# TravisWheelerLab/BATH

Hardware: AMD Instinct MI355X
Metric: DP Gcells/s + residues/s through bathsearch pipeline at 1/2/4/8 MI355X (higher is better)
Workload: dtype u8/i16 integer scores (SSV: exact binary16), f32 Forward

## Files before the change

### bath_amd/csrc/bath_pipeline.hip

```cpp
#include <algorithm>
#include <cmath>
#include <cstring>
#include <cstdlib>
#include <map>
#include <thread>

#include "bath_common.hpp"
#include "bath_kernels.hpp"
#include "bath_launch.hpp"
#include "host_model.hpp"

using namespace bath;

namespace bath {

static const double kLog2 = 0.69314718055994529;

enum { FLAG_VIT_RUN = 1, FLAG_HAS_WIN = 2 };

struct Counters {
  int cand_count, todo_msv, todo_vit, todo_ssvb, todo_vit2, todo_fwd, win_count, overflow;
  int todo_lb;
  int fwd_next;
  unsigned long long n_orfs, orf_res;
  unsigned long long n_past_msv, n_past_bias, n_past_vit, n_past_fwd;
  unsigned long long pos_past_msv, pos_past_bias, pos_past_vit, pos_past_fwd;
  unsigned long long res_vit, res_fwd;
  unsigned long long res_seen;
};

struct Params {
  double F1, F2, F3, F4;
  int do_bias, fs_pipe, minlen;
  float evparam[BATH_NEVPARAM];
};

template <int NR, int G>
__global__ __launch_bounds__(256, NR <= 76 ? 4 : 1) void ssv_orf_kernel(const uint8_t *__restrict__ aa, const OrfRec *__restrict__ orfs, const int *__restrict__ n_orfs_dev,
                                                      SeqView dna, const int16_t *__restrict__ cost_tab, int row_bytes,
                                                      const int16_t *__restrict__ emit_thresh, int thresh_max,
                                                      Cand cand, int cand_cap, Counters *__restrict__ ctr) {
  extern __shared__ __attribute__((aligned(16))) char lds[];
  {
    const int n32 = kSsvRows * row_bytes / 4;
    const uint32_t *src = reinterpret_cast<const uint32_t *>(cost_tab);
    uint32_t *dst = reinterpret_cast<uint32_t *>(lds);
    for (int i = threadIdx.x; i < n32; i += blockDim.x) dst[i] = src[i];
  }
  __syncthreads();
  constexpr int TPW = 64 / G;
  const int64_t n_orfs = *n_orfs_dev;
  const int lane = threadIdx.x & 63;
  const int grank = SsvGroups<G>::rank(lane);
  const char *tile = lds + grank * (4 * NR);
  const unsigned tile_addr = (unsigned)(size_t)(__attribute__((address_space(3))) const char *)tile;
  const int64_t wave0 = ((int64_t)blockIdx.x * blockDim.x + threadIdx.x) >> 6;
  const int64_t nwaves = ((int64_t)gridDim.x * blockDim.x) >> 6;
  const s16x2 fl = {0, 0};
  for (int64_t tb = wave0 * TPW; tb < n_orfs; tb += nwaves * TPW) {
    const int64_t t = tb + SsvGroups<G>::slot(lane);
    const bool live = t < n_orfs;
    OrfRec rec{0, 0, 0};
    if (live) rec = orfs[t];
    const int L = rec.len_sf & 0x0fffffff;
    const uint8_t *s = aa + rec.aa_off;
    const int Lw = wave_max_i32(L);
    s16x2 reg[NR];
#pragma unroll
    for (int r = 0; r < NR; r++) reg[r] = fl;
    s16x2 xE = fl, xE2 = fl;
    uint64_t qnext = (0 < L) ? *reinterpret_cast<const uint64_t *>(s) : 0x1d1d1d1d1d1d1d1dull;
    for (int i0 = 0; i0 < Lw; i0 += 8) {
      const uint64_t q = qnext;
      qnext = (i0 + 8 < L) ? *reinterpret_cast<const uint64_t *>(s + i0 + 8) : 0x1d1d1d1d1d1d1d1dull;
      const int nrow = min(8, Lw - i0);
      for (int h = 0; h < 2; h++) {
        const uint32_t qh = h ? (uint32_t)(q >> 32) : (uint32_t)q;
        const int nh = min(4, nrow - 4 * h);
        for (int j = 0; j < nh; j++) {
          int x = (int)__builtin_amdgcn_ubfe(qh, 8 * j, 8);
          x = (i0 + 4 * h + j < L) ? x : kRowReset;
          const unsigned carry = ssv_carry<NR, G>(reg, grank);
          ssv_row_pipe<NR, 3>(reg, xE, xE2, tile_addr + __umul24((unsigned)x, (unsigned)row_bytes), carry);
        }
      }
    }
    xE = ssv_max3(xE, xE2, xE2);
    const int v = ssv_group_max<G>(xE);
    if (dna.context) {
      unsigned long long r = 0;
      if (live && grank == 0) {
        const int sf = (int)((unsigned)rec.len_sf >> 28);
        const int64_t w = rec.w;
        const int startj = (int32_t)(rec.aa_off - (2 * dna.off[w] + 96 * w + (int64_t)sf * orf_stream_pitch(dna.len[w])));
        const int C = dna.context[w], start_s = sf % 3 + 3 * startj + 1;
        if (sf < 3 ? (start_s + 3 * L - 1 < C) : (dna.len[w] - start_s + 1 < C)) r = (unsigned long long)L;
      }
      if (__ballot(r != 0)) { for (int d = 32; d >= 1; d >>= 1) r += __shfl_xor(r, d, 64); if (lane == 0) atomicAdd(&ctr->res_seen, r); }
    }
    if (live && grank == 0 && v >= (int)emit_thresh[min(L, thresh_max)]) {
      const int sf = (int)((unsigned)rec.len_sf >> 28);
      const int64_t w = rec.w;
      const int64_t stream = 2 * dna.off[w] + 96 * w + (int64_t)sf * orf_stream_pitch(dna.len[w]);
      const int startj = (int32_t)(rec.aa_off - stream);
      bool seen = false;
      if (dna.context) {
        const int C = dna.context[w], start_s = sf % 3 + 3 * startj + 1;
        seen = sf < 3 ? (start_s + 3 * L - 1 < C) : (dna.len[w] - start_s + 1 < C);
      }
      const int slot = seen ? cand_cap + 1 : atomicAdd(&ctr->cand_count, 1);
      if (seen) {
      } else if (slot < cand_cap) {
        cand.window[slot] = w; cand.sf[slot] = sf; cand.startj[slot] = startj; cand.len[slot] = L;
        cand.v[slot] = (int16_t)min(v, 32767); cand.off[slot] = rec.aa_off;
      } else atomicOr(&ctr->overflow, 1);
    }
  }
}

__device__ __forceinline__ double d_gumbel_surv(double x, double mu, double lambda) {
  const double ey = -exp(-lambda * (x - mu));
  if (fabs(ey) < 5e-9) return -ey;
  return 1.0 - exp(ey);
}
__device__ __forceinline__ double d_exp_surv(double x, double mu, double lambda) { return (x < mu) ? 1.0 : exp(-lambda * (x - mu)); }

__device__ __forceinline__ int cand_classify(const Cand &cand, int c, int tjb, const MsvConsts &mc) {
  float sc = 0.f;
  const int st = ssv_classify(cand.v[c], tjb, mc, &sc);
  cand.usc[c] = sc; cand.msv_status[c] = st; cand.stage[c] = 0; cand.flags[c] = 0;
  cand.vfsc[c] = -INFINITY; cand.fwdsc[c] = -INFINITY; cand.vit_status[c] = 0; cand.filtersc[c] = 0.f; cand.P[c] = 1.0;
  cand.kminmax[2 * c] = 1 << 30; cand.kminmax[2 * c + 1] = 0;
  return st;
}

template <int NL, int NS, int CAP>
struct BlockTally {
  int n[NL > 0 ? NL : 1], base[NL > 0 ? NL : 1];
  unsigned long long sum[NS > 0 ? NS : 1];
  int32_t ids[NL > 0 ? NL : 1][NL > 0 ? CAP : 1];
};
template <int NL, int NS>
struct TallyOut {
  int32_t *list[NL > 0 ? NL : 1]; int *count[NL > 0 ? NL : 1];
  unsigned long long *sum[NS > 0 ? NS : 1];
};
template <int NL, int NS, int CAP>
__device__ __forceinline__ void tally_reset(BlockTally<NL, NS, CAP> &t) {
  if ((int)threadIdx.x < NL) t.n[threadIdx.x] = 0;
  if ((int)threadIdx.x < NS) t.sum[threadIdx.x] = 0ull;
  __syncthreads();
}
template <int NL, int NS, int CAP>
__device__ __forceinline__ void tally_add(BlockTally<NL, NS, CAP> &t, int k, unsigned long long v) { atomicAdd(&t.sum[k], v); }
template <int NL, int NS, int CAP>
__device__ __forceinline__ void tally_push(BlockTally<NL, NS, CAP> &t, int l, int32_t id) { t.ids[l][atomicAdd(&t.n[l], 1)] = id; }
template <int NL, int NS, int CAP>
__device__ __forceinline__ bool tally_lists_full(BlockTally<NL, NS, CAP> &t) {
  bool full = false;
  __syncthreads();
#pragma unroll
  for (int l = 0; l < NL; l++) full |= t.n[l] > CAP - (int)blockDim.x;
  __syncthreads();
  return full;
}
template <int NL, int NS, int CAP>
__device__ __forceinline__ void tally_write_lists(BlockTally<NL, NS, CAP> &t, const TallyOut<NL, NS> &o) {
  if (NL == 0) return;
  __syncthreads();
#pragma unroll
  for (int l = 0; l < NL; l++) if ((int)threadIdx.x == l && t.n[l] > 0) t.base[l] = atomicAdd(o.count[l], t.n[l]);
  __syncthreads();
#pragma unroll
  for (int l = 0; l < NL; l++) {
    const int n = t.n[l], b = t.base[l];
    for (int i = threadIdx.x; i < n; i += blockDim.x) o.list[l][b + i] = t.ids[l][i];
  }
  __syncthreads();
  if ((int)threadIdx.x < NL) t.n[threadIdx.x] = 0;
  __syncthreads();
}
template <int NL, int NS, int CAP>
__device__ __forceinline__ void tally_finish(BlockTally<NL, NS, CAP> &t, const TallyOut<NL, NS> &o) {
  tally_write_lists(t, o);
  if (NL == 0) __syncthreads();
#pragma unroll
  for (int k = 0; k < NS; k++) if ((int)threadIdx.x == k && t.sum[k] != 0ull) atomicAdd(o.sum[k], t.sum[k]);
}

__global__ __launch_bounds__(256) void classify_kernel(Cand cand, int cand_cap, Counters *__restrict__ ctr, const uint8_t *__restrict__ tjb_tab, MsvConsts mc,
                                                       int32_t *__restrict__ todo_msv) {
  __shared__ BlockTally<1, 0, 512> tally;
  tally_reset(tally);
  const TallyOut<1, 0> out{{todo_msv}, {&ctr->todo_msv}, {nullptr}};
  const int ncand = min(ctr->cand_count, cand_cap);
  for (int c0 = blockIdx.x * blockDim.x; c0 < ncand; c0 += gridDim.x * blockDim.x) {
    if (tally_lists_full(tally)) tally_write_lists(tally, out);
    const int c = c0 + threadIdx.x;
    if (c < ncand && cand_classify(cand, c, tjb_tab[cand.len[c]], mc) == BATH_ENORESULT) tally_push(tally, 0, c);
  }
  tally_finish(tally, out);
}

struct F1Tables { const float *eo, *nullsc, *p1, *lt1, *lt2; };
enum { F1_TODO_VIT = 0, F1_TODO_SSVB = 1, F1_NL = 2 };
enum { F1_N_MSV = 0, F1_POS_MSV, F1_N_BIAS, F1_POS_BIAS, F1_RES_VIT, F1_NS };
__device__ __forceinline__ TallyOut<F1_NL, F1_NS> f1_tally_out(Counters *__restrict__ ctr, int32_t *__restrict__ todo_vit, int32_t *__restrict__ todo_ssvb) {
  return TallyOut<F1_NL, F1_NS>{{todo_vit, todo_ssvb}, {&ctr->todo_vit, &ctr->todo_ssvb},
                                {&ctr->n_past_msv, &ctr->pos_past_msv, &ctr->n_past_bias, &ctr->pos_past_bias, &ctr->res_vit}};
}
template <int CAP>
__device__ __forceinline__ void cand_f1_bias(const Cand &cand, int c, BlockTally<F1_NL, F1_NS, CAP> &tally, const Params &p, const uint8_t *__restrict__ pool, int M,
                                             const float *s_eo , const F1Tables &t) {
  const int L = cand.len[c];
  const float usc = cand.usc[c];
  const float nullsc = t.nullsc[L];
  cand.nullsc[c] = nullsc;
  float seqsc = (float)((double)(usc - nullsc) / kLog2);
  double P = d_gumbel_surv(seqsc, p.evparam[0], p.evparam[1]);
  cand.P[c] = P;
  if (P > p.F1) return;
  tally_add(tally, F1_N_MSV, 1ull); tally_add(tally, F1_POS_MSV, (unsigned long long)L * 3ull);
  cand.stage[c] = 1;
  float filtersc = nullsc;
  if (p.do_bias) {
    filtersc = bias_forward(pool + cand.off[c], L, M, s_eo, t.p1[L]);
    filtersc = (filtersc + t.lt1[L]) + t.lt2[L];
    seqsc = (float)((double)(usc - filtersc) / kLog2);
    P = d_gumbel_surv(seqsc, p.evparam[0], p.evparam[1]);
    cand.P[c] = P; cand.filtersc[c] = filtersc;
    if (P > p.F1) return;
  }
  cand.filtersc[c] = filtersc;
  tally_add(tally, F1_N_BIAS, 1ull); tally_add(tally, F1_POS_BIAS, (unsigned long long)L * 3ull);
  cand.stage[c] = 2;
  if (P > p.F2) { cand.flags[c] |= FLAG_VIT_RUN; tally_push(tally, F1_TODO_VIT, c); tally_add(tally, F1_RES_VIT, (unsigned long long)L); }
  else tally_push(tally, F1_TODO_SSVB, c);
}

__global__ __launch_bounds__(256) void f1_bias_kernel(Cand cand, int cand_cap, Counters *__restrict__ ctr, Params p, const uint8_t *__restrict__ pool, int M, F1Tables t,
                                                      int32_t *__restrict__ todo_vit, int32_t *__restrict__ todo_ssvb) {
  __shared__ float s_eo[kKp * 2];
  __shared__ BlockTally<F1_NL, F1_NS, 512> tally;
  for (int i = threadIdx.x; i < kKp * 2; i += blockDim.x) s_eo[i] = t.eo[i];
  tally_reset(tally);
  const TallyOut<F1_NL, F1_NS> out = f1_tally_out(ctr, todo_vit, todo_ssvb);
  const int ncand = min(ctr->cand_count, cand_cap);
  for (int c0 = blockIdx.x * blockDim.x; c0 < ncand; c0 += gridDim.x * blockDim.x) {
    if (tally_lists_full(tally)) tally_write_lists(tally, out);
    const int c = c0 + threadIdx.x;
    if (c < ncand) cand_f1_bias(cand, c, tally, p, pool, M, s_eo, t);
  }
  tally_finish(tally, out);
}

template <int NR>
__global__ __launch_bounds__(256, 4) void msv_stage_kernel(Cand cand, int cand_cap, Counters *__restrict__ ctr,
                                                           const int16_t *__restrict__ cost_tab , int row_bytes,
                                                           const uint8_t *__restrict__ tjb_tab, MsvConsts mc, Params p, const uint8_t *__restrict__ pool, int M,
                                                           F1Tables t, int32_t *__restrict__ todo_vit, int32_t *__restrict__ todo_ssvb) {
  extern __shared__ __attribute__((aligned(16))) char lds[];
  __shared__ float s_eo[kKp * 2];
  __shared__ BlockTally<F1_NL, F1_NS, 256> tally;
  const int ncand = min(ctr->cand_count, cand_cap);
  if ((int64_t)blockIdx.x * blockDim.x >= ncand) return;
  {
    const int n32 = kSsvRows * row_bytes / 4;
    const uint32_t *src = reinterpret_cast<const uint32_t *>(cost_tab);
    uint32_t *dst = reinterpret_cast<uint32_t *>(lds);
    for (int i = threadIdx.x; i < n32; i += blockDim.x) dst[i] = src[i];
    for (int i = threadIdx.x; i < kKp * 2; i += blockDim.x) s_eo[i] = t.eo[i];
  }
  tally_reset(tally);
  const int64_t job = (int64_t)blockIdx.x * blockDim.x + threadIdx.x;
  const bool live = job < ncand;
  const int c = live ? (int)job : 0;
  const int L = live ? cand.len[c] : 0;
  const int tjb = tjb_tab[L];
  const bool rescore = live && cand_classify(cand, c, tjb, mc) == BATH_ENORESULT;
  const int Lr = rescore ? L : 0;
  const uint8_t *s = pool + (rescore ? cand.off[c] : 0);
  bool overflow = false;
  const int xJ = msv_lane_rows<NR>(lds, row_bytes, s, Lr, wave_max_i32(Lr), (uint8_t)((int8_t)tjb + (int8_t)mc.tbm), mc, &overflow);
  if (rescore) {
    if (overflow) { cand.usc[c] = INFINITY; cand.msv_status[c] = BATH_ERANGE; }
    else { cand.usc[c] = msv_lane_score(xJ, tjb, mc); cand.msv_status[c] = BATH_OK; }
  }
  if (live) cand_f1_bias(cand, c, tally, p, pool, M, s_eo, t);
  tally_finish(tally, f1_tally_out(ctr, todo_vit, todo_ssvb));
}

template <int C>
__global__ __launch_bounds__(256) void ssv_bath_kernel(Cand cand, const Counters *__restrict__ ctr, const int32_t *__restrict__ todo,
                                                       const uint8_t *__restrict__ pool, int M, const uint8_t *__restrict__ rb, int rb_stride,
                                                       const uint8_t *__restrict__ ssv_scores, const uint8_t *__restrict__ tjb_tab,
                                                       const float *__restrict__ nullsc_tab, MsvConsts mc, double invP_f1,
                                                       WindowRec *__restrict__ wins, int win_cap, Counters *__restrict__ ctrw) {
  const int lane = threadIdx.x & 63;
  const int64_t wid = ((int64_t)blockIdx.x * blockDim.x + threadIdx.x) >> 6;
  const int64_t nw = ((int64_t)gridDim.x * blockDim.x) >> 6;
  const int ntodo = ctr->todo_ssvb;
  const int Q = max(2, ((M - 1) / 16) + 1);
  for (int64_t job = wid; job < ntodo; job += nw) {
    const int c = todo[job];
    const int L = cand.len[c];
    const uint8_t *s = pool + cand.off[c];
    const int tjb = tjb_tab[L];
    const float nullsc = nullsc_tab[L];
    const int sc_thresh = (uint8_t)(int)ceil((((double)nullsc + ((double)(float)invP_f1 * kLog2) + 3.0) * (double)mc.scale_b) + mc.base + mc.tec + tjb);
    const int tjbm = (uint8_t)((int8_t)tjb + (int8_t)mc.tbm);
    const int xB = satu8(mc.base - tjbm);
    int kmin = 1 << 30, kmax = 0;
    int dp[C];
#pragma unroll
    for (int k = 0; k < C; k++) dp[k] = 0;
    const int ph = threadIdx.x & 63;
    int rbuf = (ph < L) ? (int)s[ph] : 0, rnext = 0;
    for (int i = 1; i <= L; i++) {
      const int j = (i - 1) & 63;
      if (j == 0) { const int q = i - 1 + 64 + ph; rnext = (q < L) ? (int)s[q] : 0; }
      const int x = min(__builtin_amdgcn_readlane(rbuf, j), kKp - 1);
      if (j == 63) rbuf = rnext;
      const uint8_t *row = rb + (size_t)x * rb_stride;
      int prev = wave_shr1_i32(dp[C - 1], 0);
      int xE = 0;
#pragma unroll
      for (int k = 0; k < C; k++) {
        const int node = lane * C + k + 1;
        const int cost = (node <= M) ? (int)row[node] : 255;
        int sv = max(prev, xB);
        sv = satu8(sv + mc.bias);
        sv = satu8(sv - cost);
        prev = dp[k];
        dp[k] = sv;
        xE = max(xE, sv);
      }
      xE = wave_max_i32(xE);
      if (xE >= sc_thresh) {
        int rank = 1 << 30;
#pragma unroll
        for (int k = 0; k < C; k++) {
          const int node = lane * C + k + 1;
          if (node <= M && dp[k] == xE) rank = min(rank, ((node - 1) % Q) * 16 + (node - 1) / Q);
        }
        rank = wave_min_i32(rank);
        int end = (rank / 16) + Q * (rank % 16) + 1;
        int rem_sc = xE;
#pragma unroll
        for (int k = 0; k < C; k++) dp[k] = 0;
        int start = end, target_end = i, target_start = i;
        int sc = rem_sc;
        while (rem_sc > mc.base - tjb - mc.tbm && start >= 1 && target_start >= 1) {
          rem_sc -= mc.bias - (int)ssv_scores[(size_t)start * kKp + min((int)s[target_start - 1], kKp - 1)];
          --start; --target_start;
        }
        start++; target_start++;
        int k = end + 1, n = target_end + 1, max_end = target_end, max_sc = sc, since = 0;
        while (k < M && n <= L) {
          sc += mc.bias - (int)ssv_scores[(size_t)k * kKp + min((int)s[n - 1], kKp - 1)];
          if (sc >= max_sc) { max_sc = sc; max_end = n; since = 0; }
          else { since++; if (since == 5) break; }
          k++; n++;
        }
        end += (max_end - target_end);
        target_end = max_end;
        float ret = ((float)(max_sc - tjb) - (float)mc.base);
        ret /= mc.scale_b;
        ret = (float)((double)ret - 3.0);
        if (lane == 0) {
          const int slot = atomicAdd(&ctrw->win_count, 1);
          if (slot < win_cap) wins[slot] = WindowRec{c, target_start, end, end - start + 1, ret};
        }
        kmin = min(kmin, start); kmax = max(kmax, end);
        i = target_end;
        { const int base = i & ~63; rbuf = (base + ph < L) ? (int)s[base + ph] : 0; rnext = (base + 64 + ph < L) ? (int)s[base + 64 + ph] : 0; }
      }
    }
    if (lane == 0) { cand.kminmax[2 * c] = kmin; cand.kminmax[2 * c + 1] = kmax; }
  }
}

__device__ __forceinline__ float local_compo_x(const uint8_t *ssv_scores, int M, int base_b, float scale_b, const float *bgf, int k_start, int k_end, int x) {
  const int k_len = k_end - k_start + 1;
  if (k_len < 20) { k_start -= (20 - k_len) / 2; k_end += (20 - k_len) / 2; }
  k_start = max(1, k_start); k_end = min(M, k_end);
  float acc = 0.0f;
  for (int k = k_start; k <= k_end; k++) {
    const float lo = ((float)base_b - (float)ssv_scores[(size_t)k * kKp + x]) / scale_b;
    acc += bgf[x] * expf(lo);
  }
  return acc;
}
__device__ void local_compo_finish(float *compo , const float *bgf, float *eo );
__device__ void local_compo_eo(const uint8_t *ssv_scores, int M, int base_b, float scale_b, const float *bgf, int k_start, int k_end, float *eo ) {
  float compo[20];
  for (int x = 0; x < 20; x++) compo[x] = local_compo_x(ssv_scores, M, base_b, scale_b, bgf, k_start, k_end, x);
  local_compo_finish(compo, bgf, eo);
}
__device__ void local_compo_finish(float *compo, const float *bgf, float *eo) {
  float sum = 0.f, cc = 0.f;
  for (int x = 0; x < 20; x++) { const float y = compo[x] - cc; const float t = sum + y; cc = (t - sum) - y; sum = t; }
  if (sum != 0.0f) for (int x = 0; x < 20; x++) compo[x] /= sum;
  else for (int x = 0; x < 20; x++) compo[x] = 1.0f / 20.0f;
  for (int x = 0; x < 20; x++) { eo[2 * x] = bgf[x] / bgf[x]; eo[2 * x + 1] = compo[x] / bgf[x]; }
  eo[2 * 20] = eo[2 * 20 + 1] = 1.0f; eo[2 * 27] = eo[2 * 27 + 1] = 1.0f; eo[2 * 28] = eo[2 * 28 + 1] = 1.0f;
  const int mem[6][2] = {{2, 11}, {7, 9}, {3, 13}, {8, 8}, {1, 1}, {-1, -1}};
  for (int dx = 0; dx < 6; dx++) {
    float n0 = 0.f, n1 = 0.f, den = 0.f;
    if (dx == 5) { for (int y = 0; y < 20; y++) { n0 += bgf[y]; n1 += compo[y]; den += bgf[y]; } }
    else {
      const int a = min(mem[dx][0], mem[dx][1]), b = max(mem[dx][0], mem[dx][1]);
      n0 += bgf[a]; n1 += compo[a]; den += bgf[a];
      if (b != a) { n0 += bgf[b]; n1 += compo[b]; den += bgf[b]; }
    }
    eo[2 * (21 + dx)] = den > 0.f ? n0 / den : 0.f;
    eo[2 * (21 + dx) + 1] = den > 0.f ? n1 / den : 0.f;
  }
}
// ... 106 lines not shown
  __shared__ BlockTally<1, 1, 512> tally;
  tally_reset(tally);
  const TallyOut<1, 1> out{{todo_fwd}, {&ctr->todo_fwd}, {&ctr->res_fwd}};
  const int ntodo = ctr->todo_vit2;
  for (int job0 = blockIdx.x * blockDim.x; job0 < ntodo; job0 += gridDim.x * blockDim.x) {
    if (tally_lists_full(tally)) tally_write_lists(tally, out);
    const int job = job0 + threadIdx.x;
    if (job >= ntodo) continue;
    const int c = todo_vit2[job];
    const float seqsc = (float)((double)(cand.vfsc[c] - cand.filtersc[c]) / kLog2);
    const double P = d_gumbel_surv(seqsc, p.evparam[2], p.evparam[3]);
    cand.P[c] = P;
    if (P > p.F2) { cand.stage[c] = 2; continue; }
    cand.stage[c] = 3;
    tally_push(tally, 0, c); tally_add(tally, 0, (unsigned long long)cand.len[c]);
  }
  tally_finish(tally, out);
}

__global__ __launch_bounds__(256) void final_kernel(Cand cand, Counters *__restrict__ ctr, Params p, const int32_t *__restrict__ todo_fwd) {
  __shared__ BlockTally<0, 2, 1> tally;
  tally_reset(tally);
  const TallyOut<0, 2> out{{nullptr}, {nullptr}, {&ctr->n_past_fwd, &ctr->pos_past_fwd}};
  const int ntodo = ctr->todo_fwd;
  for (int job = blockIdx.x * blockDim.x + threadIdx.x; job < ntodo; job += gridDim.x * blockDim.x) {
    const int c = todo_fwd[job];
    const float seqsc = (float)((double)(cand.fwdsc[c] - cand.filtersc[c]) / kLog2);
    const double P = d_exp_surv(seqsc, p.evparam[4], p.evparam[5]);
    cand.P[c] = P;
    if (P > (p.fs_pipe ? p.F4 : p.F3)) continue;
    cand.stage[c] = 4;
    tally_add(tally, 0, 1ull);
    if (!p.fs_pipe) tally_add(tally, 1, (unsigned long long)cand.len[c] * 3ull);
  }
  tally_finish(tally, out);
}

__global__ void copy_count_kernel(const int *src, int64_t *dst) { *dst = *src; }

}


namespace bath {

static int ssv_classify_host(int v, int tjb, const MsvConsts &c, float *sc) {
  if (tjb + c.tbm + c.tec + c.bias >= 127) return BATH_ENORESULT;
  unsigned xE = (v >= -1 - c.bias) ? 255u : (unsigned)(v + 256);
  if ((int)xE >= 255 - c.bias) { *sc = INFINITY; return (c.base - tjb - c.tbm < 128) ? BATH_ENORESULT : BATH_ERANGE; }
  xE = (xE + (unsigned)(c.base - tjb - c.tbm) - 128u) & 0xffffu;
  if ((int)xE >= 255 - c.bias) { *sc = INFINITY; return BATH_ERANGE; }
  unsigned xJ = (xE - (unsigned)c.tec) & 0xffffu;
  if ((int)xJ > c.base) return BATH_ENORESULT;
  float r = ((float)((int)xJ - tjb) - (float)c.base);
  r /= c.scale_b;
  r = (float)((double)r - 3.0);
  *sc = r;
  return BATH_OK;
}

static void build_emit_table(const bath_hip_oprofile *om, double F1, int maxlen, std::vector<int16_t> &tab) {
  const MsvConsts mc = msv_consts(om);
  tab.assign((size_t)maxlen + 1, (int16_t)32767);
  for (int len = 0; len <= maxlen; len++) {
    const int tjb = om->lt.h_tjb[len];
    const float nullsc = om->lt.h_nullsc[len];
    auto keep = [&](int v) {
      float usc = 0.f;
      if (ssv_classify_host(v, tjb, mc, &usc) != BATH_OK) return true;
      const float seqsc = (float)((double)(usc - nullsc) / kLog2);
      return !(gumbel_surv(seqsc, om->evparam[0], om->evparam[1]) > F1);
    };
    if (!keep(127)) continue;
    int lo = -128, hi = 127;
    while (lo < hi) { const int mid = lo + (hi - lo) / 2; if (keep(mid)) hi = mid; else lo = mid + 1; }
    tab[(size_t)len] = (int16_t)lo;
  }
}

static int ensure_emit_table(bath_hip_ctx *ctx, const bath_hip_oprofile *om, double F1, int maxlen) {
  std::lock_guard<std::mutex> lock(om->grow_mu);
  if (om->emit_F1 == F1 && om->emit_maxlen >= maxlen && om->d_emit) return BATH_OK;
  std::vector<int16_t> tab;
  build_emit_table(om, F1, maxlen, tab);
  if (om->d_emit) om->retired.push_back(om->d_emit);
  om->d_emit = nullptr;
  BATH_HIP_TRY(ctx, hipMalloc((void **)&om->d_emit, tab.size() * sizeof(int16_t) + 64));
  BATH_HIP_TRY(ctx, hipMemcpy(om->d_emit, tab.data(), tab.size() * sizeof(int16_t), hipMemcpyHostToDevice));
  om->emit_F1 = F1; om->emit_maxlen = maxlen;
  return BATH_OK;
}

int build_compo_terms(bath_hip_ctx *ctx, bath_hip_oprofile *om) {
  BATH_HIP_TRY(ctx, hipMalloc((void **)&om->d_compo_terms, (size_t)(20 * 256 + 20) * sizeof(float) + 64));
  float *d_bgf = om->d_compo_terms + 20 * 256;
  BATH_HIP_TRY(ctx, hipMemcpyAsync(d_bgf, kAminoBg, 20 * sizeof(float), hipMemcpyHostToDevice, ctx->stream));
  hipLaunchKernelGGL(compo_terms_kernel, dim3(20), dim3(256), 0, ctx->stream, d_bgf, (int)om->base_b, om->scale_b, om->d_compo_terms);
  BATH_HIP_TRY(ctx, hipGetLastError());
  BATH_HIP_TRY(ctx, hipStreamSynchronize(ctx->stream));
  return BATH_OK;
}

static int wave_grid_blocks(bath_hip_ctx *ctx) { return ctx->prop.multiProcessorCount * 8; }

struct PipelineWork {
  Cand cand;
  int cand_cap = 0;
  uint8_t *pool = nullptr;
  int32_t *todo_msv = nullptr, *todo_vit = nullptr, *todo_ssvb = nullptr, *todo_vit2 = nullptr, *todo_fwd = nullptr, *todo_sorted = nullptr;
  int *len_bins = nullptr;
  WindowRec *wins = nullptr;
  int win_cap = 0;
  Counters *ctr = nullptr;
};

template <class T>
static T *carve(char *&p, size_t n) {
  T *r = reinterpret_cast<T *>(p);
  p += (n * sizeof(T) + 255) / 256 * 256;
  return r;
}

static size_t layout(PipelineWork &w, char *base, int cap, int win_cap) {
  char *p = base;
  const size_t n = (size_t)cap;
  w.cand_cap = cap; w.win_cap = std::max(2 * cap, win_cap);
  if (win_cap == 0) {
    static const int forced = [] { const char *e = std::getenv("BATH_HIP_TEST_WINCAP"); return e ? std::atoi(e) : 0; }();
    if (forced > 0) w.win_cap = forced;
  }
  w.ctr = carve<Counters>(p, 1);
  w.cand.window = carve<int64_t>(p, n); w.cand.off = carve<int64_t>(p, n); w.cand.P = carve<double>(p, n);
  w.cand.sf = carve<int32_t>(p, n); w.cand.startj = carve<int32_t>(p, n); w.cand.len = carve<int32_t>(p, n);
  w.cand.msv_status = carve<int32_t>(p, n); w.cand.vit_status = carve<int32_t>(p, n); w.cand.fwd_status = carve<int32_t>(p, n); w.cand.stage = carve<int32_t>(p, n);
  w.cand.flags = carve<int32_t>(p, n); w.cand.kminmax = carve<int32_t>(p, 2 * n);
  w.cand.usc = carve<float>(p, n); w.cand.nullsc = carve<float>(p, n); w.cand.filtersc = carve<float>(p, n);
  w.cand.vfsc = carve<float>(p, n); w.cand.fwdsc = carve<float>(p, n);
  w.cand.v = carve<int16_t>(p, n);
  w.todo_msv = carve<int32_t>(p, n); w.todo_vit = carve<int32_t>(p, n); w.todo_ssvb = carve<int32_t>(p, n);
  w.todo_vit2 = carve<int32_t>(p, n); w.todo_fwd = carve<int32_t>(p, n); w.todo_sorted = carve<int32_t>(p, n);
  w.len_bins = carve<int>(p, 2048);
  w.wins = carve<WindowRec>(p, (size_t)w.win_cap);
  return (size_t)(p - base);
}

}

extern "C" int bath_selftest_compo_terms(int base_b, float scale_b, float *terms) {
  if (!terms || !(scale_b > 0.f)) return BATH_EINVAL;
  for (int x = 0; x < 20; x++)
    for (int sc = 0; sc < 256; sc++) terms[x * 256 + sc] = bath::compo_term(kAminoBg[x], base_b, sc, scale_b);
  return BATH_OK;
}

extern "C" void bath_pipeline_params_default(bath_pipeline_params *p, int fs_pipe) {
  p->F1 = 0.02; p->F2 = 1e-3; p->F3 = 1e-5; p->F4 = 5e-4;
  p->do_biasfilter = 1; p->fs_pipe = fs_pipe; p->min_orf_len = 20; p->ncbi_table = 1;
  p->nres_before = 0;
  p->do_null2 = 1; p->std_pipe = 1; p->strands = BATH_STRAND_BOTH; p->initiator = BATH_INIT_ANY;
  p->inc_by_E = 1; p->seed = 42; p->T = 0.0;
}

extern "C" int bath_hip_pipeline_timings(const bath_hip_ctx *ctx, int max, const char **names, float *ms, int64_t *launches) {
  int n = std::min<int>(max, (int)ctx->timings.size());
  for (int i = 0; i < n; i++) { names[i] = ctx->timings[i].name; ms[i] = ctx->timings[i].ms; launches[i] = ctx->timings[i].launches; }
  return n;
}

namespace bath {
struct FilterState {
  PipelineWork W;
  Counters hc{};
  const uint8_t *d_ssvsc = nullptr;
  const float *d_bgf = nullptr;
  OrfTablesDev tt{};
};
}

__global__ __launch_bounds__(64) void fwd_keep_offsets_kernel(const int32_t *__restrict__ todo, const int *__restrict__ ntodo_dev, const int32_t *__restrict__ len,
                                                              int64_t *__restrict__ off, int64_t cap) {
  const int lane = threadIdx.x, n = *ntodo_dev;
  int64_t base = 0;
  for (int j0 = 0; j0 < n; j0 += 64) {
    const int j = j0 + lane;
    const int sid = j < n ? todo[j] : -1;
    const int64_t v = sid >= 0 ? ((int64_t)len[sid] + 1) * 6 : 0;
    int64_t incl = v;
    for (int d = 1; d < 64; d <<= 1) { const int64_t u = __shfl_up(incl, d, 64); if (lane >= d) incl += u; }
    if (sid >= 0) off[sid] = (base + incl <= cap) ? base + incl - v : (int64_t)-1;
    base += __shfl(incl, 63, 64);
  }
}

static int cascade_model_ok(bath_hip_ctx *ctx, const bath_hip_oprofile *om) {
  if (om->M <= kCascadeMaxNodes) return BATH_OK;
  ctx->set_error("the filter cascade supports models up to " + std::to_string(kCascadeMaxNodes) + " nodes (this one has " + std::to_string(om->M) + ")");
  return BATH_EINVAL;
}

static int launch_ssv_bath(bath_hip_ctx *ctx, hipStream_t stream, const bath_hip_oprofile *om, const Cand &cand, Counters *ctr, const int32_t *todo, const uint8_t *pool,
                           const uint8_t *ssv_scores, const MsvConsts &mc, double invP, WindowRec *wins, int win_cap);

static int run_filters(bath_hip_ctx *ctx, const bath_hip_oprofile *om, const bath_hip_seqs *dna,
                       const bath_pipeline_params *prm, bath_pipeline_stats *stats,
                       const bath_orf_result **results, int64_t *n_results, FilterState *state) {
  if (!ctx || !om || !dna || !prm) return BATH_EINVAL;
  if (cascade_model_ok(ctx, om) != BATH_OK) return BATH_EINVAL;
  BATH_HIP_TRY(ctx, hipSetDevice(ctx->device));
  if (n_results) *n_results = 0;
  if (results) *results = nullptr;
  if (stats) std::memset(stats, 0, sizeof *stats);
  const int64_t nwin = dna->n;
  if (nwin == 0) return BATH_OK;
  const int M = om->M;
  const int max_orf = dna->maxlen / 3 + 1;
  int st = om->ensure_len_tables(max_orf);
  if (st != BATH_OK) return st;

  OrfTablesDev tt{};
  if (prm->strands < 0 || prm->strands > 2 || prm->initiator < 0 || prm->initiator > 2) { ctx->set_error("bath_pipeline_params: strands / initiator out of range"); return BATH_EINVAL; }
  if ((st = orf_tables_upload(ctx, prm->ncbi_table, &tt, prm->initiator)) != BATH_OK) return st;
  if ((st = ensure_emit_table(ctx, om, prm->F1, max_orf)) != BATH_OK) return st;
  DevBuf &b_tabs = ctx->scratch[Scratch::kSsvScoreTable], &b_work = ctx->scratch[Scratch::kCascadeWork];
  const size_t ssv_bytes = (size_t)(M + 1) * kKp;
  const size_t tabs_bytes = 8192 + ssv_bytes + 256 + 20 * 4 + 256;
  if (tabs_bytes > b_tabs.cap) ctx->tabs_uid = 0;
  BATH_HIP_TRY(ctx, b_tabs.reserve(tabs_bytes));
  char *tp = b_tabs.as<char>();
  const int16_t *d_emit = om->d_emit;
  uint8_t *d_ssvsc = reinterpret_cast<uint8_t *>(tp); tp += (ssv_bytes + 255) / 256 * 256;
  float *d_bgf = reinterpret_cast<float *>(tp);
  if (ctx->tabs_uid != om->uid || ctx->tabs_ptr != b_tabs.p) {
    std::vector<uint8_t> ssv_scores(ssv_bytes, 0);
    bath_hip_oprofile_get_ssv_scores(om, ssv_scores.data());
    BATH_HIP_TRY(ctx, hipMemcpyAsync(d_ssvsc, ssv_scores.data(), ssv_scores.size(), hipMemcpyHostToDevice, ctx->stream));
    BATH_HIP_TRY(ctx, hipMemcpyAsync(d_bgf, kAminoBg, 20 * sizeof(float), hipMemcpyHostToDevice, ctx->stream));
    BATH_HIP_TRY(ctx, hipStreamSynchronize(ctx->stream));
    ctx->tabs_uid = om->uid; ctx->tabs_ptr = b_tabs.p;
  }

  Params P{};
  P.F1 = prm->F1; P.F2 = prm->F2; P.F3 = prm->F3; P.F4 = prm->F4;
  P.do_bias = prm->do_biasfilter; P.fs_pipe = prm->fs_pipe; P.minlen = prm->min_orf_len;
  std::memcpy(P.evparam, om->evparam, sizeof P.evparam);
  const MsvConsts mc = msv_consts(om);
  const double invP_f1 = gumbel_invsurv(prm->F1, om->evparam[0], om->evparam[1]);
  VitWindowArgs wa{};
  wa.invP_vit = (double)(float)gumbel_invsurv(prm->F2, om->evparam[2], om->evparam[3]);
  wa.invP_msv = (double)(float)gumbel_invsurv(prm->F2, om->evparam[0], om->evparam[1]);

  if (dna->cache_minlen != prm->min_orf_len) {
    int64_t nres_c = 0, max_orfs_c = 0;
    for (int64_t i = 0; i < nwin; i++) {
      const int n = dna->h_len[i];
      if (n < 15) continue;
      nres_c += 2 * (int64_t)(n - (dna->h_context.empty() ? 0 : dna->h_context[(size_t)i]));
      max_orfs_c += 6 * (int64_t)((n / 3 + 1) / (prm->min_orf_len + 1) + 1);
    }
    dna->cache_minlen = prm->min_orf_len; dna->cache_nres = nres_c; dna->cache_max_orfs = max_orfs_c;
  }
  const int64_t nres = prm->strands == BATH_STRAND_BOTH ? dna->cache_nres : dna->cache_nres / 2;
  const int64_t max_orfs = dna->cache_max_orfs;
  if (max_orfs >= (int64_t)INT32_MAX) { ctx->set_error("DNA block too large for one pipeline call (ORF list indices are 32-bit): split it"); return BATH_EINVAL; }
  int64_t cap = std::max<int64_t>(4096, (int64_t)((double)max_orfs * std::min(1.0, prm->F1 * 4.0 + 0.01)));
  cap = std::min<int64_t>(cap, std::max<int64_t>(max_orfs, 4096));
  {
    static const int forced = [] { const char *e = std::getenv("BATH_HIP_TEST_CANDCAP"); return e ? std::atoi(e) : 0; }();
    if (forced > 0) cap = forced;
  }

  if ((st = orf_tiles_ensure(ctx, dna)) != BATH_OK) return st;
  const size_t nent = (size_t)dna->ntiles * 6;
  DevBuf &b_aa = ctx->scratch[Scratch::kOrfAminoPool], &b_slots = ctx->scratch[Scratch::kOrfSlots], &b_orfs = ctx->scratch[Scratch::kOrfRecords], &b_misc = ctx->scratch[Scratch::kOrfMisc];
  BATH_HIP_TRY(ctx, b_aa.reserve(orf_aa_bytes(dna)));
  BATH_HIP_TRY(ctx, b_slots.reserve(((size_t)dna->ntiles * (size_t)orf_slot_cap(prm->min_orf_len) + 64) * 8));
  BATH_HIP_TRY(ctx, b_orfs.reserve((size_t)(max_orfs + 64) * sizeof(OrfRec)));
  BATH_HIP_TRY(ctx, b_misc.reserve((5 * nent + kOrfMiscInts) * sizeof(int32_t)));
  OrfBuffers ob{};
  orf_buffers_carve(&ob, b_aa.p, b_slots.p, b_orfs.p, b_misc.p, nent);

  const int NRk = om->NR;
  const size_t ssv_shmem = (size_t)kSsvRows * om->ssv_row_bytes;
  if ((st = ssv_table_fits(ctx, om)) != BATH_OK) return st;
  const int dec_blocks = ctx->prop.multiProcessorCount * 4;

  std::vector<hipEvent_t> &ev = ctx->ev_pool;
  while (ev.size() < 12) { hipEvent_t e; BATH_HIP_TRY(ctx, hipEventCreate(&e)); ev.push_back(e); }

  PipelineWork W;
  Counters hc{};
  int win_need = 0;
  for (int attempt = 0;; attempt++) {
    size_t need = layout(W, nullptr, (int)cap, win_need);
    BATH_HIP_TRY(ctx, b_work.reserve(need + 4096));
    layout(W, b_work.as<char>(), (int)cap, win_need);
    W.pool = b_aa.as<uint8_t>();
    BATH_HIP_TRY(ctx, hipMemsetAsync(W.ctr, 0, sizeof(Counters), ctx->stream));
    SeqView cv{W.pool, W.cand.off, W.cand.len, cap};

    int e = 0;
    BATH_HIP_TRY(ctx, hipEventRecord(ev[e++], ctx->stream));
    if ((st = launch_orf_scan(ctx, dna, tt, prm->min_orf_len, ob, &W.ctr->n_orfs, &W.ctr->orf_res, prm->strands)) != BATH_OK) return st;
    BATH_HIP_TRY(ctx, hipEventRecord(ev[e++], ctx->stream));
    {
      const int blocks = ctx->prop.multiProcessorCount * 4;
      const int ssv_threads = 256;
      bool launched = false;
#define BATH_ORF_CASE(N, GG)                                                                                                     \
  if (!launched && NRk == N && om->G == GG) {                                                                                    \
    if (ssv_shmem > 64 * 1024) (void)bath::allow_max_lds((const void *)ssv_orf_kernel<N, GG>); \
    hipLaunchKernelGGL((ssv_orf_kernel<N, GG>), dim3(blocks), dim3(ssv_threads), ssv_shmem, ctx->stream, W.pool, ob.sorted, ob.ntotal,                  \
                       dna->view(), om->d_ssv, om->ssv_row_bytes, d_emit, max_orf, W.cand, W.cand_cap, W.ctr);                   \
    launched = true;                                                                                                             \
  }
      BATH_SSV_SHAPES(BATH_ORF_CASE)
#undef BATH_ORF_CASE
      if (!launched) { ctx->set_error("SSV kernel: no tile shape for this model length"); return BATH_EINVAL; }
      BATH_HIP_TRY(ctx, hipGetLastError());
    }
    BATH_HIP_TRY(ctx, hipEventRecord(ev[e++], ctx->stream));
    const bool few_cands = dna->total < lane_min_nt(), few_msv = dna->total < 2 * lane_min_nt();
    const F1Tables f1t{om->d_bias_eo, om->lt.d_nullsc, om->lt.d_p1, om->lt.d_lt1, om->lt.d_lt2};
    const bool msv_stage = !few_msv && msv_stage_supported(om);
    if (msv_stage) {
      bool launched = false;
#define BATH_MSV_STAGE_CASE(N, ...)                                                                                                         \
  if (!launched && NRk == N) {                                                                                                              \
    hipLaunchKernelGGL((msv_stage_kernel<N>), dim3((unsigned)((W.cand_cap + 255) / 256)), dim3(256), ssv_shmem, ctx->stream, W.cand, W.cand_cap, W.ctr, om->d_msv, \
                       om->ssv_row_bytes, om->lt.d_tjb, mc, P, W.pool, M, f1t, W.todo_vit, W.todo_ssvb);                                      \
    launched = true;                                                                                                                        \
  }
      BATH_MSV_LANE_NR(BATH_MSV_STAGE_CASE)
#undef BATH_MSV_STAGE_CASE
      if (!launched) { ctx->set_error("MSV stage kernel: no tile shape for this model length"); return BATH_EINVAL; }
      BATH_HIP_TRY(ctx, hipGetLastError());
      BATH_HIP_TRY(ctx, hipEventRecord(ev[e++], ctx->stream));
      BATH_HIP_TRY(ctx, hipEventRecord(ev[e++], ctx->stream));
    } else {
      hipLaunchKernelGGL(classify_kernel, dim3(dec_blocks), dim3(256), 0, ctx->stream, W.cand, W.cand_cap, W.ctr, om->lt.d_tjb, mc, W.todo_msv);
      BATH_HIP_TRY(ctx, hipGetLastError());
      if ((st = launch_msv_wave(ctx, om, cv, W.todo_msv, cap, W.cand.usc, W.cand.msv_status, &W.ctr->todo_msv, !few_msv)) != BATH_OK) return st;
      BATH_HIP_TRY(ctx, hipEventRecord(ev[e++], ctx->stream));
      hipLaunchKernelGGL(f1_bias_kernel, dim3(dec_blocks), dim3(256), 0, ctx->stream, W.cand, W.cand_cap, W.ctr, P, W.pool, M, f1t, W.todo_vit, W.todo_ssvb);
      BATH_HIP_TRY(ctx, hipGetLastError());
      BATH_HIP_TRY(ctx, hipEventRecord(ev[e++], ctx->stream));
    }
    wa.d_filtersc = W.cand.filtersc; wa.d_ssv_scores = d_ssvsc; wa.d_wins = W.wins; wa.d_win_count = &W.ctr->win_count; wa.win_cap = W.win_cap;
    wa.d_kminmax = W.cand.kminmax;
    auto launch_ssvb = [&](hipStream_t stream) -> int {
      return launch_ssv_bath(ctx, stream, om, W.cand, W.ctr, W.todo_ssvb, W.pool, d_ssvsc, mc, invP_f1, W.wins, W.win_cap);
    };
    bool ssvb_done = false;
    if (vit_lane_supported(om) && !few_cands) {
      if ((st = launch_vit_sorted(ctx, om, cv, W.todo_vit, cap, &W.ctr->todo_vit, W.cand.len, W.len_bins, W.todo_sorted, W.cand.vfsc, W.cand.vit_status, &wa,
                                  launch_ssvb)) != BATH_OK) return st;
      ssvb_done = true;
    } else if ((st = launch_vit_wave(ctx, om, cv, W.todo_vit, cap, W.cand.vfsc, W.cand.vit_status, &wa, &W.ctr->todo_vit)) != BATH_OK) return st;
    BATH_HIP_TRY(ctx, hipEventRecord(ev[e++], ctx->stream));
    if (!ssvb_done && (st = launch_ssvb(ctx->stream)) != BATH_OK) return st;
    BATH_HIP_TRY(ctx, hipGetLastError());
    BATH_HIP_TRY(ctx, hipEventRecord(ev[e++], ctx->stream));
    hipLaunchKernelGGL(post_vit_kernel, dim3(dec_blocks), dim3(256), 0, ctx->stream, W.cand, W.cand_cap, W.ctr, P, W.todo_msv , W.todo_fwd);
    if (P.do_bias) {
      DevBuf &b_compo = ctx->scratch[Scratch::kLocalCompoSums];
      BATH_HIP_TRY(ctx, b_compo.reserve((size_t)W.cand_cap * 20 * 4 + 256));
      float *d_compo = b_compo.as<float>();
      hipLaunchKernelGGL(local_compo_kernel, dim3(16384), dim3(64), 0, ctx->stream, W.cand, W.ctr, M, d_ssvsc, om->d_compo_terms, W.todo_msv, d_compo);
      hipLaunchKernelGGL(post_vit_local_kernel, dim3(std::max(1, dec_blocks)), dim3(64), 0, ctx->stream, W.cand, W.ctr, P, W.pool, M, d_bgf, d_compo,
                         om->lt.d_p1, om->lt.d_lt1, om->lt.d_lt2, W.todo_msv, W.todo_vit2, W.todo_fwd);
    }
    BATH_HIP_TRY(ctx, hipGetLastError());
    if ((st = launch_vit_wave(ctx, om, cv, W.todo_vit2, cap, W.cand.vfsc, W.cand.vit_status, nullptr, &W.ctr->todo_vit2)) != BATH_OK) return st;
    hipLaunchKernelGGL(post_vit2_kernel, dim3(64), dim3(256), 0, ctx->stream, W.cand, W.ctr, P, W.todo_vit2, W.todo_fwd);
    BATH_HIP_TRY(ctx, hipGetLastError());
    BATH_HIP_TRY(ctx, hipEventRecord(ev[e++], ctx->stream));
    ctx->fwd_rows_kept = nullptr; ctx->fwd_rows_off = nullptr;
    float *d_keep = nullptr; int64_t *d_keep_off = nullptr;
    if (ctx->keep_fwd_rows) {
      constexpr int64_t kKeepFloats = (int64_t)8 << 20;
      DevBuf &b_rows = ctx->scratch[Scratch::kCascadeFwdRows], &b_roff = ctx->scratch[Scratch::kCascadeFwdRowOffsets];
      BATH_HIP_TRY(ctx, b_rows.reserve((size_t)kKeepFloats * sizeof(float) + 64)); BATH_HIP_TRY(ctx, b_roff.reserve((size_t)cap * sizeof(int64_t) + 64));
      d_keep = b_rows.as<float>(); d_keep_off = b_roff.as<int64_t>();
      hipLaunchKernelGGL(fwd_keep_offsets_kernel, dim3(1), dim3(64), 0, ctx->stream, W.todo_fwd, &W.ctr->todo_fwd, W.cand.len, d_keep_off, kKeepFloats);
      BATH_HIP_TRY(ctx, hipGetLastError());
    }
    const bool fwd_group = !d_keep && fwd_group_supported(om) && ctx->fwd_group != 2;
    if (fwd_group) {
      if ((st = launch_len_sort(ctx, W.todo_fwd, &W.ctr->todo_fwd, W.cand.len, W.len_bins, W.todo_sorted)) != BATH_OK) return st;
      if ((st = launch_fwd_group(ctx, om, cv, W.todo_sorted, cap, &W.ctr->todo_fwd, &W.ctr->fwd_next, W.cand.fwdsc, W.cand.fwd_status)) != BATH_OK) return st;
    } else if ((st = launch_fwd_wave(ctx, om, cv, W.todo_fwd, cap, W.cand.fwdsc, W.cand.fwd_status, &W.ctr->todo_fwd, d_keep, d_keep_off)) != BATH_OK) return st;
    const int64_t fwd_launches = (d_keep ? 1 : 0) + (fwd_group ? 4 : 1) + 1;
    if (d_keep) { ctx->fwd_rows_kept = d_keep; ctx->fwd_rows_off = d_keep_off; }
    hipLaunchKernelGGL(final_kernel, dim3(dec_blocks), dim3(256), 0, ctx->stream, W.cand, W.ctr, P, W.todo_fwd);
    BATH_HIP_TRY(ctx, hipGetLastError());
    BATH_HIP_TRY(ctx, hipEventRecord(ev[e++], ctx->stream));

    BATH_HIP_TRY(ctx, hipMemcpyAsync(&hc, W.ctr, sizeof(Counters), hipMemcpyDeviceToHost, ctx->stream));
    BATH_HIP_TRY(ctx, hipStreamSynchronize(ctx->stream));
    if (hc.overflow || hc.cand_count > cap || hc.win_count > W.win_cap) {
      if (attempt >= 4) { ctx->set_error("candidate / window buffers overflowed repeatedly"); return BATH_EMEM; }
      if (hc.overflow || hc.cand_count > cap) cap = std::max<int64_t>(cap * 2, (int64_t)hc.cand_count + 1024);
      if (hc.win_count > W.win_cap) win_need = hc.win_count + hc.win_count / 4 + 1024;
      continue;
    }
    static const char *names[] = {"translate_orfs", "ssv_f1", "classify_msv", "f1_bias", "viterbi_windows", "ssv_windows", "post_vit", "forward_final"};
    const int64_t launches[] = {4, 1, msv_stage ? 1 : 2, msv_stage ? 0 : 1, 4, 1, 3, fwd_launches};
    ctx->timings.clear();
    for (int i = 0; i + 1 < e; i++) {
      float ms = 0.f;
      BATH_HIP_TRY(ctx, hipEventElapsedTime(&ms, ev[i], ev[i + 1]));
      ctx->timings.push_back(StageTiming{names[i], ms, launches[i]});
    }
    break;
  }

  if (stats) {
    stats->nres = nres; stats->n_orfs = (int64_t)hc.n_orfs;
    stats->n_past_msv = (int64_t)hc.n_past_msv; stats->n_past_bias = (int64_t)hc.n_past_bias;
    stats->n_past_vit = (int64_t)hc.n_past_vit; stats->n_past_fwd = (int64_t)hc.n_past_fwd;
    stats->pos_past_msv = (int64_t)hc.pos_past_msv; stats->pos_past_bias = (int64_t)hc.pos_past_bias;
    stats->pos_past_vit = (int64_t)hc.pos_past_vit; stats->pos_past_fwd = (int64_t)hc.pos_past_fwd;
    stats->cells_msv = (int64_t)(hc.orf_res - hc.res_seen) * M; stats->cells_vit = (int64_t)hc.res_vit * M; stats->cells_fwd = (int64_t)hc.res_fwd * M;
  }

  if (results) {
    bath_orf_result *d_rec = nullptr;
    int64_t nrec = 0;
    if (dna->n > (int64_t)UINT32_MAX || dna->maxlen / 3 >= (1 << 28)) { ctx->set_error("block too large for the ORF records' sort key (2^32 windows, 805 Mnt per window)"); return BATH_ERANGE; }
    if ((st = build_orf_records(ctx, W.cand, hc.cand_count, dna->is_part ? dna->first_window : 0, &d_rec, &nrec)) != BATH_OK) return st;
    ctx->d_records = d_rec; ctx->n_records = nrec;
    if (!dna->is_part) {
      BATH_HIP_TRY(ctx, ctx->results_pinned.reserve((size_t)std::max<int64_t>(nrec, 1) * sizeof(bath_orf_result)));
      if (nrec > 0) BATH_HIP_TRY(ctx, hipMemcpyAsync(ctx->results_pinned.p, d_rec, (size_t)nrec * sizeof(bath_orf_result), hipMemcpyDeviceToHost, ctx->stream));
      BATH_HIP_TRY(ctx, hipStreamSynchronize(ctx->stream));
      *results = ctx->results_pinned.as<bath_orf_result>();
    } else *results = nullptr;
    if (n_results) *n_results = nrec;
  } else if (n_results) *n_results = (int64_t)hc.n_past_msv;
  if (state) { state->W = W; state->hc = hc; state->d_ssvsc = d_ssvsc; state->d_bgf = d_bgf; state->tt = tt; }
  return BATH_OK;
}

static int pipeline_lane_count(const bath_hip_seqs *dna) {
  const char *e = std::getenv("BATH_HIP_LANES");
  const int forced = e ? std::atoi(e) : 0;
  if (forced > 0) return (int)std::min<int64_t>(forced, std::max<int64_t>(dna->n, 1));
  if (dna->is_part || dna->n < 8) return 1;
  int K = (dna->total >= ((int64_t)1 << 28)) ? 2 : 1;
  const int64_t by_size = (dna->total + ((int64_t)1 << 34) - 1) >> 34;
  if (by_size > K) K = (int)std::min<int64_t>(by_size, std::max<int64_t>(dna->n, 1));
  return K;
}

static int ensure_parts(bath_hip_ctx *ctx, const bath_hip_seqs *dna, int K) {
  if ((int)dna->parts.size() == K) return BATH_OK;
  for (bath_hip_seqs *p : dna->parts) bath_hip_seqs_destroy(p);
  dna->parts.clear();
  int64_t w0 = 0;
  for (int k = 0; k < K; k++) {
    int64_t w1 = w0;
    if (k == K - 1) w1 = dna->n;
    else {
      const int64_t target = dna->total_aligned / K * (k + 1);
      w1 = std::lower_bound(dna->h_off.begin() + w0, dna->h_off.end(), target) - dna->h_off.begin();
      w1 = std::max(w1, std::min(w0 + 1, dna->n));
    }
    bath_hip_seqs *p = new bath_hip_seqs();
    p->ctx = ctx; p->is_part = true; p->first_window = w0; p->n = w1 - w0;
    const int64_t base = w0 < dna->n ? dna->h_off[(size_t)w0] : dna->total_aligned;
    p->h_off.resize((size_t)p->n); p->h_len.assign(dna->h_len.begin() + w0, dna->h_len.begin() + w1);
    for (int64_t i = 0; i < p->n; i++) {
      p->h_off[(size_t)i] = dna->h_off[(size_t)(w0 + i)] - base;
      p->maxlen = std::max(p->maxlen, p->h_len[(size_t)i]);
      p->total += p->h_len[(size_t)i];
    }
    p->total_aligned = (w1 < dna->n ? dna->h_off[(size_t)w1] : dna->total_aligned) - base;
    p->d_data = dna->d_data + base;
    p->d_len = dna->d_len + w0;
    if (dna->d_context) { p->d_context = dna->d_context + w0; p->h_context.assign(dna->h_context.begin() + w0, dna->h_context.begin() + w1); }
    dna->parts.push_back(p);
    if (hipMalloc((void **)&p->d_off, (size_t)std::max<int64_t>(p->n, 1) * sizeof(int64_t)) != hipSuccess) { ctx->set_error("hipMalloc (block parts)"); return BATH_EMEM; }
    if (p->n > 0 && hipMemcpy(p->d_off, p->h_off.data(), (size_t)p->n * sizeof(int64_t), hipMemcpyHostToDevice) != hipSuccess) { ctx->set_error("hipMemcpy (block parts)"); return BATH_EFAIL; }
    w0 = w1;
  }
  return BATH_OK;
}

template <class After>
static int run_filters_lanes(bath_hip_ctx *ctx, const bath_hip_oprofile *om, const bath_hip_seqs *dna,
                             const bath_pipeline_params *prm, bath_pipeline_stats *stats,
                             const bath_orf_result **results, int64_t *n_results, std::vector<FilterState> *states, After after) {
  if (!ctx || !om || !dna || !prm) return BATH_EINVAL;
  if (cascade_model_ok(ctx, om) != BATH_OK) return BATH_EINVAL;
  const int K = pipeline_lane_count(dna);
  if (K <= 1) {
    states->assign(1, FilterState{});
    int st = run_filters(ctx, om, dna, prm, stats, results, n_results, &(*states)[0]);
    if (st != BATH_OK) return st;
    return after(0, ctx, dna, (*states)[0]);
  }
  BATH_HIP_TRY(ctx, hipSetDevice(ctx->device));
  int st = om->ensure_len_tables(dna->maxlen / 3 + 1);
  if (st != BATH_OK) return st;
  if ((st = ensure_emit_table(ctx, om, prm->F1, dna->maxlen / 3 + 1)) != BATH_OK) return st;
  while ((int)ctx->lanes.size() < K) {
    bath_hip_ctx *lane = nullptr;
    if ((st = bath_hip_init(ctx->device, &lane)) != BATH_OK) { ctx->set_error("cannot create a pipeline lane"); return st; }
    mark_internal(lane);
    int lo = 0, hi = 0;
    if (hipDeviceGetStreamPriorityRange(&lo, &hi) == hipSuccess && lo != hi) {
      (void)hipStreamDestroy(lane->stream);
      if (hipStreamCreateWithPriority(&lane->stream, hipStreamNonBlocking, ctx->lanes.empty() ? hi : lo) != hipSuccess) { ctx->set_error("hipStreamCreateWithPriority"); return BATH_EFAIL; }
    }
    ctx->lanes.push_back(lane);
  }
  for (bath_hip_ctx *lane : ctx->lanes) { lane->fs_strict = ctx->fs_strict; lane->fs_odds = ctx->fs_odds; lane->fs5_odds = ctx->fs5_odds; lane->fwd_group = ctx->fwd_group; }
  if ((st = ensure_parts(ctx, dna, K)) != BATH_OK) return st;
  std::vector<bath_pipeline_stats> pst((size_t)K);
  std::vector<const bath_orf_result *> pres((size_t)K, nullptr);
  std::vector<int64_t> pn((size_t)K, 0);
  std::vector<int> rc((size_t)K, BATH_OK);
  states->assign((size_t)K, FilterState{});
  if (!ctx->ev_lanes) BATH_HIP_TRY(ctx, hipEventCreateWithFlags(&ctx->ev_lanes, hipEventDisableTiming));
  BATH_HIP_TRY(ctx, hipEventRecord(ctx->ev_lanes, ctx->stream));
  for (int k = 0; k < K; k++) BATH_HIP_TRY(ctx, hipStreamWaitEvent(ctx->lanes[(size_t)k]->stream, ctx->ev_lanes, 0));
  if (!ctx->lane_pool) ctx->lane_pool = new LanePool();
  ctx->lane_pool->run(K, [&](int k) {
    bath_hip_ctx *lane = ctx->lanes[(size_t)k];
    rc[(size_t)k] = run_filters(lane, om, dna->parts[(size_t)k], prm, &pst[(size_t)k], results ? &pres[(size_t)k] : nullptr, &pn[(size_t)k], &(*states)[(size_t)k]);
    if (rc[(size_t)k] == BATH_OK) rc[(size_t)k] = after(k, lane, dna->parts[(size_t)k], (*states)[(size_t)k]);
  });
  for (int k = 0; k < K; k++)
    if (rc[(size_t)k] != BATH_OK) { ctx->set_error(ctx->lanes[(size_t)k]->err); return rc[(size_t)k]; }

  bath_pipeline_stats tot{};
  int64_t ntot = 0;
  for (int k = 0; k < K; k++) {
    const bath_pipeline_stats &a = pst[(size_t)k];
    tot.nres += a.nres; tot.n_orfs += a.n_orfs; tot.n_past_msv += a.n_past_msv; tot.n_past_bias += a.n_past_bias; tot.n_past_vit += a.n_past_vit;
    tot.n_past_fwd += a.n_past_fwd; tot.pos_past_msv += a.pos_past_msv; tot.pos_past_bias += a.pos_past_bias; tot.pos_past_vit += a.pos_past_vit;
    tot.pos_past_fwd += a.pos_past_fwd; tot.cells_msv += a.cells_msv; tot.cells_vit += a.cells_vit; tot.cells_fwd += a.cells_fwd;
    ntot += pn[(size_t)k];
  }
  if (stats) *stats = tot;
  if (results) {
    BATH_HIP_TRY(ctx, ctx->results_pinned.reserve((size_t)std::max<int64_t>(ntot, 1) * sizeof(bath_orf_result)));
    bath_orf_result *dst = ctx->results_pinned.as<bath_orf_result>();
    int64_t at = 0;
    for (int k = 0; k < K; k++) {
      bath_hip_ctx *lane = ctx->lanes[(size_t)k];
      const int64_t nk = pn[(size_t)k];
      if (nk > 0) BATH_HIP_TRY(ctx, hipMemcpyAsync(dst + at, lane->d_records, (size_t)nk * sizeof(bath_orf_result), hipMemcpyDeviceToHost, lane->stream));
      at += nk;
    }
    for (int k = 0; k < K; k++) BATH_HIP_TRY(ctx, hipStreamSynchronize(ctx->lanes[(size_t)k]->stream));
    *results = dst;
  }
  if (n_results) *n_results = ntot;
  ctx->timings.clear();
  for (int k = 0; k < K; k++) {
    const std::vector<StageTiming> &t = ctx->lanes[(size_t)k]->timings;
    for (size_t i = 0; i < t.size(); i++) {
      if (k == 0) ctx->timings.push_back(t[i]);
      else if (i < ctx->timings.size()) { ctx->timings[i].ms += t[i].ms; ctx->timings[i].launches += t[i].launches; }
    }
  }
  return BATH_OK;
}

extern "C" int bath_hip_pipeline_filters(bath_hip_ctx *ctx, const bath_hip_oprofile *om, const bath_hip_seqs *dna,
                                         const bath_pipeline_params *prm, bath_pipeline_stats *stats,
                                         const bath_orf_result **results, int64_t *n_results) {
  std::vector<FilterState> states;
  return run_filters_lanes(ctx, om, dna, prm, stats, results, n_results, &states,
                           [](int, bath_hip_ctx *, const bath_hip_seqs *, const FilterState &) { return (int)BATH_OK; });
}

namespace bath {


__global__ void fs_window_gather_kernel(const uint8_t *__restrict__ dna, const FsWinDev *__restrict__ wins, int nw, const uint8_t *__restrict__ comp,
                                        uint8_t *__restrict__ pool) {
  for (int w = blockIdx.x; w < nw; w += gridDim.x) {
    const FsWinDev d = wins[w];
    const uint8_t *src = dna + d.src_off;
    uint8_t *dst = pool + d.dst_off;
    for (int i = threadIdx.x; i < d.len; i += blockDim.x) {
      const int r = d.start - 1 + i;
      dst[i] = d.strand ? comp[min((int)src[d.seq_n - 1 - r], 17)] : src[r];
    }
  }
}

__global__ void fs_bias_kernel(const uint8_t *__restrict__ pool, const FsWinDev *__restrict__ wins, int nw, const uint8_t *__restrict__ aa_full, int M,
                               const float *__restrict__ eo_global, const uint8_t *__restrict__ ssv_scores, int base_b, float scale_b,
                               const float *__restrict__ bgf, float *__restrict__ out) {
  const int t = blockIdx.x * blockDim.x + threadIdx.x;
  if (t >= 2 * nw) return;
  const int w = t >> 1, pass = t & 1;
  const FsWinDev d = wins[w];
  float eo_local[2 * kKp];
  const float *e = eo_global;
  if (pass == 1) {
    if (d.kmin > d.kmax) { out[t * 3] = out[t * 3 + 1] = out[t * 3 + 2] = -INFINITY; return; }
    local_compo_eo(ssv_scores, M, base_b, scale_b, bgf, d.kmin, d.kmax, eo_local);
    e = eo_local;
  }
  const uint8_t *s = pool + d.dst_off;
// ... 417 lines not shown
```

Measured before the change: 216.9 billion.

## Replace static grid-stride SSV ORF loop with atomic dynamic chunk claiming

The SSV ORF kernel stops giving waves a fixed grid-stride share of ORF chunks. When there are many chunks, each wave claims work from a global atomic counter instead, and sizes each claim (1-4 chunks) from the average residues per wave and from how much work is left. The goal is to balance the load when ORF lengths vary, so no wave is left holding the slow tail. In exchange it adds atomic traffic and a prefetch claim that runs before the LDS fill, plus an env var that caps the block count for testing.

New measurement: 217.1 billion (median of 4 runs). No clear change (+0.1%).

```diff
diff --git a/bath_amd/csrc/bath_pipeline.hip b/bath_amd/csrc/bath_pipeline.hip
--- a/bath_amd/csrc/bath_pipeline.hip
+++ b/bath_amd/csrc/bath_pipeline.hip
@@ -27,6 +27,7 @@
   unsigned long long pos_past_msv, pos_past_bias, pos_past_vit, pos_past_fwd;
   unsigned long long res_vit, res_fwd;
   unsigned long long res_seen;
+  int ssv_next;
 };
 
 struct Params {
@@ -35,12 +36,28 @@
   float evparam[BATH_NEVPARAM];
 };
 
+constexpr int kSsvStrideRounds = 8;
 template <int NR, int G>
 __global__ __launch_bounds__(256, NR <= 76 ? 4 : 1) void ssv_orf_kernel(const uint8_t *__restrict__ aa, const OrfRec *__restrict__ orfs, const int *__restrict__ n_orfs_dev,
                                                       SeqView dna, const int16_t *__restrict__ cost_tab, int row_bytes,
                                                       const int16_t *__restrict__ emit_thresh, int thresh_max,
                                                       Cand cand, int cand_cap, Counters *__restrict__ ctr) {
   extern __shared__ __attribute__((aligned(16))) char lds[];
+  constexpr int TPW = 64 / G;
+  const int lane = threadIdx.x & 63;
+  const int64_t n_orfs = *n_orfs_dev;
+  const int nchunks = (int)((n_orfs + TPW - 1) / TPW);
+  const int nwaves = (int)((gridDim.x * blockDim.x) >> 6);
+  const int claim_rows = (int)((float)ctr->orf_res / (8.f * TPW * nwaves));
+  auto claim_size = [&](int pos, int rows) {
+    const int left = nchunks - pos;
+    const int by_end = 1 + (left >= 2 * nwaves) + (left >= 3 * nwaves) + (left >= 4 * nwaves);
+    const int by_rows = 1 + (2 * rows <= claim_rows) + (3 * rows <= claim_rows) + (4 * rows <= claim_rows);
+    return min(by_end, by_rows);
+  };
+  const bool claims = nchunks > kSsvStrideRounds * nwaves;
+  int nclaim = 1, taken = 0;
+  if (claims && lane == 0) taken = atomicAdd(&ctr->ssv_next, nclaim);
   {
     const int n32 = kSsvRows * row_bytes / 4;
     const uint32_t *src = reinterpret_cast<const uint32_t *>(cost_tab);
@@ -48,23 +65,23 @@
     for (int i = threadIdx.x; i < n32; i += blockDim.x) dst[i] = src[i];
   }
   __syncthreads();
-  constexpr int TPW = 64 / G;
-  const int64_t n_orfs = *n_orfs_dev;
-  const int lane = threadIdx.x & 63;
   const int grank = SsvGroups<G>::rank(lane);
   const char *tile = lds + grank * (4 * NR);
   const unsigned tile_addr = (unsigned)(size_t)(__attribute__((address_space(3))) const char *)tile;
-  const int64_t wave0 = ((int64_t)blockIdx.x * blockDim.x + threadIdx.x) >> 6;
-  const int64_t nwaves = ((int64_t)gridDim.x * blockDim.x) >> 6;
   const s16x2 fl = {0, 0};
-  for (int64_t tb = wave0 * TPW; tb < n_orfs; tb += nwaves * TPW) {
-    const int64_t t = tb + SsvGroups<G>::slot(lane);
+  int chunk = __builtin_amdgcn_readfirstlane(claims ? taken : (int)((blockIdx.x * blockDim.x + threadIdx.x) >> 6)), chunk_end = min(chunk + nclaim, nchunks);
+  while (chunk < nchunks) {
+    const int64_t t = (int64_t)chunk * TPW + SsvGroups<G>::slot(lane);
     const bool live = t < n_orfs;
     OrfRec rec{0, 0, 0};
     if (live) rec = orfs[t];
     const int L = rec.len_sf & 0x0fffffff;
     const uint8_t *s = aa + rec.aa_off;
     const int Lw = wave_max_i32(L);
+    if (claims && chunk + 1 == chunk_end) {
+      nclaim = claim_size(chunk_end, __builtin_amdgcn_readfirstlane(Lw));
+      if (lane == 0) taken = atomicAdd(&ctr->ssv_next, nclaim);
+    }
     s16x2 reg[NR];
 #pragma unroll
     for (int r = 0; r < NR; r++) reg[r] = fl;
@@ -114,6 +131,10 @@
         cand.window[slot] = w; cand.sf[slot] = sf; cand.startj[slot] = startj; cand.len[slot] = L;
         cand.v[slot] = (int16_t)min(v, 32767); cand.off[slot] = rec.aa_off;
       } else atomicOr(&ctr->overflow, 1);
+    }
+    if (++chunk == chunk_end) {
+      chunk = claims ? __builtin_amdgcn_readfirstlane(taken) : chunk - 1 + nwaves;
+      chunk_end = min(chunk + nclaim, nchunks);
     }
   }
 }
@@ -826,7 +847,11 @@
     if ((st = launch_orf_scan(ctx, dna, tt, prm->min_orf_len, ob, &W.ctr->n_orfs, &W.ctr->orf_res, prm->strands)) != BATH_OK) return st;
     BATH_HIP_TRY(ctx, hipEventRecord(ev[e++], ctx->stream));
     {
-      const int blocks = ctx->prop.multiProcessorCount * 4;
+      int blocks = ctx->prop.multiProcessorCount * 4;
+      {
+        static const int forced = [] { const char *e = std::getenv("BATH_HIP_TEST_SSV_BLOCKS"); return e ? std::atoi(e) : 0; }();
+        if (forced > 0) blocks = std::min(blocks, forced);
+      }
       const int ssv_threads = 256;
       bool launched = false;
 #define BATH_ORF_CASE(N, GG)                                                                                                     \
```
